# gfacciol/mgm

Measured on AMD Instinct MI355X. Metric: disparity-volumes/sec (W*H*L cost volume -> 8-dir MGM -> WTA+vfit), higher is better.
Workload: dtype f32

## Files before the change

### mgm_amd/csrc/mgm_ctx.hip

```cpp
#include "mgm_host.h"

long long mgm::tune_num(const char *key, long long dflt)
{
#ifdef MGM_HIP_RELEASE
    (void)key;
    return dflt;
#else
    static const std::vector<std::pair<std::string, long long>> table = [] {
        std::vector<std::pair<std::string, long long>> t;
        if (const char *e = getenv("MGM_HIP_TUNE")) {
            std::string s(e);
            size_t i = 0;
            while (i < s.size()) {
                size_t j = s.find(',', i);
                if (j == std::string::npos) j = s.size();
                const std::string item = s.substr(i, j - i);
                const size_t q = item.find('=');
                if (q != std::string::npos && q > 0) t.emplace_back(item.substr(0, q), atoll(item.c_str() + q + 1));
                i = j + 1;
            }
        }
        return t;
    }();
    for (const auto &kv : table)
        if (kv.first == key) return kv.second;
    std::string legacy = "MGM_HIP_";
    for (const char *q = key; *q; q++) legacy += (char)toupper((unsigned char)*q);
    if (const char *e = getenv(legacy.c_str())) return atoll(e);
    return dflt;
#endif
}

const DevSwitches &dev()
{
    static const DevSwitches d = [] {
        auto on = [](const char *n) { return tune_num(n, 1) != 0; };
        return DevSwitches{on("c8"), on("lazy_f32"), on("pad"), (int)tune_num("subv", 1), (int)tune_num("deep", -1),
                           (int)tune_num("wg_per_cu", 0), (int)tune_num("xflags", 0), (int)tune_num("strips", -1), (int)tune_num("xcdq", -1),
                           (int)tune_num("xcdq_k", -1), on("w2"), on("oneb"), 64ll * tune_num("lr_pad", 67)};
    }();
    return d;
}
long long lr_pad_floats() { return dev().lr_pad; }
const WtaSwitches &wta_switches()
{
    static const WtaSwitches w{(int)tune_num("wta_prune_ppw", 2), (int)tune_num("wta_prune_wg", 0), (int)tune_num("wta_wg_per_cu", 0),
                               tune_num("wta_packed", 1) != 0, tune_num("wta_wide4", 1) != 0, tune_num("wta_quad", 1) != 0,
                               (int)tune_num("wta_right_seg", 0)};
    return w;
}

int fail(mgm_ctx *c, int code, const std::string &msg)
{
    if (c) c->err = msg;
    return code;
}
int hipfail(mgm_ctx *c, hipError_t e, const char *what)
{
    (void)hipGetLastError();
    return fail(c, MGM_ERR_HIP, std::string(what) + ": " + hipGetErrorString(e));
}
#define HIPCHK(c, call)                                          \
    do {                                                         \
        hipError_t e__ = (call);                                 \
        if (e__ != hipSuccess) return hipfail((c), e__, #call);  \
    } while (0)

hipError_t dev_malloc(void **p, size_t bytes)
{
    const hipError_t e = hipMalloc(p, bytes);
    if (e != hipSuccess) {
        *p = nullptr;
        (void)hipGetLastError();
    }
    return e;
}

int reserve(mgm_ctx *c, Buf &b, size_t bytes)
{
    if (bytes <= b.cap) return MGM_OK;
    if (b.p) {
        HIPCHK(c, hipStreamSynchronize(c->stream));
        HIPCHK(c, hipFree(b.p));
        b.p = nullptr;
        b.cap = 0;
    }
    hipError_t e = dev_malloc(&b.p, bytes);
    if (e != hipSuccess) {
        return fail(c, MGM_ERR_NOMEM, std::string("hipMalloc(") + std::to_string(bytes) + "): " + hipGetErrorString(e));
    }
    b.cap = bytes;
    return MGM_OK;
}

int ensure_words(mgm_ctx *c)
{
    const void *before = c->words.p;
    if (int r = reserve(c, c->words, sizeof(unsigned) * (size_t)kCtrlWordsTotal)) return r;
    if (c->words.p != before) HIPCHK(c, hipMemsetAsync(c->words.p, 0, c->words.cap, c->stream));
    return MGM_OK;
}
int read_word(mgm_ctx *c, const unsigned *dev, unsigned *out)
{
    HIPCHK(c, hipMemcpyAsync(c->h_words + kHostFlag, dev, sizeof(unsigned), hipMemcpyDeviceToHost, c->stream));
    HIPCHK(c, hipStreamSynchronize(c->stream));
    *out = c->h_words[kHostFlag];
    return MGM_OK;
}

int distance_index(const char *n)
{
    static const char *t[] = {"ad", "sd", "census", "ncc", "btad", "btsd", nullptr};
    int r = 0;
    for (int i = 0; t[i]; i++)
        if (n && !strcmp(n, t[i])) r = i;
    return r;
}
int prefilter_index(const char *n)
{
    static const char *t[] = {"none", "census", "sobelx", "gblur", nullptr};
    int r = 0;
    for (int i = 0; t[i]; i++)
        if (n && !strcmp(n, t[i])) r = i;
    return r;
}
int refinement_index(const char *n)
{
    static const char *t[] = {"none", "vfit", "parabola", "cubic", "parabolaOCV", nullptr};
    int r = 0;
    for (int i = 0; t[i]; i++)
        if (n && !strcmp(n, t[i])) r = i;
    return r;
}

int watch_launch(mgm_ctx *c)
{
    HIPCHK(c, hipMemcpyAsync(c->h_words + kHostWatchdog, ctrl_word(c, kWordWatchdog), sizeof(unsigned), hipMemcpyDeviceToHost, c->stream));
    c->pending_check = true;
    return MGM_OK;
}
int check_watchdog(mgm_ctx *c, bool block)
{
    if (!c->pending_check) return MGM_OK;
    if (block) HIPCHK(c, hipStreamSynchronize(c->stream));
    else if (hipStreamQuery(c->stream) != hipSuccess) return MGM_OK;
    c->pending_check = false;
    if (c->h_words[kHostWatchdog] != 0) {
        c->h_words[kHostWatchdog] = 0;
        if (c->words.p) (void)hipMemsetAsync(ctrl_word(c, kWordWatchdog), 0, sizeof(unsigned), c->stream);
        forget_hand_regions(c);
        return fail(c, MGM_ERR_INTERNAL, "pass kernel watchdog: inter-band hand-off timed out");
    }
    return MGM_OK;
}

bool pipe_uses(const mgm_ctx *c, const void *obj)
{
    if (!c || !obj) return false;
    for (const auto &q : c->pend) {
        for (const mgm_cv *x : q.C) if (x == obj) return true;
        for (const mgm_img *x : q.w8) if (x == obj) return true;
        for (const mgm_img *x : q.out) if (x == obj) return true;
        for (const mgm_img *x : q.outcost) if (x == obj) return true;
    }
    return false;
}

static std::vector<Buf *> workspace_bufs(mgm_ctx *c)
{
    std::vector<Buf *> bufs = {&c->lr, &c->hand.buf, &c->hand2, &c->handm, &c->exact_mins, &c->exact_scratch, &c->census_u, &c->census_v, &c->dbg, &c->stmp, &c->ones8,
                               &c->lr_rel, &c->hand_rel.buf, &c->lmin, &c->wta_stats, &c->wvals, &c->speckle, &c->holes};
    for (int v = 0; v < kMaxBatch; v++) bufs.insert(bufs.end(), {&c->padf[v], &c->pad8[v], &c->wsel[v]});
    return bufs;
}
static void release(Buf &b) { if (b.p) (void)hipFree(b.p), b = Buf{}; }

extern "C" {

const char *mgm_version(void) { return "mgm-hip 0.1 (gfx950)"; }

int mgm_ctx_create(int device, mgm_ctx **out)
{
    if (!out) return MGM_ERR_INVALID;
    *out = nullptr;
    int n = 0;
    if (hipGetDeviceCount(&n) != hipSuccess || n <= 0 || device < 0 || device >= n) return MGM_ERR_HIP;
    if (hipSetDevice(device) != hipSuccess) return MGM_ERR_HIP;
    hipDeviceProp_t prop;
    if (hipGetDeviceProperties(&prop, device) != hipSuccess) return MGM_ERR_HIP;
    if (strncmp(prop.gcnArchName, "gfx950", 6) != 0) return MGM_ERR_HIP;
    mgm_ctx *c = new mgm_ctx();
    c->device = device;
    c->num_cu = prop.multiProcessorCount > 0 ? prop.multiProcessorCount : 256;
    if (hipStreamCreateWithFlags(&c->stream, hipStreamNonBlocking) != hipSuccess) {
        delete c;
        return MGM_ERR_HIP;
    }
    if (hipHostMalloc((void **)&c->h_words, kHostWords * sizeof(unsigned), hipHostMallocDefault) != hipSuccess) {
        (void)hipStreamDestroy(c->stream);
        delete c;
        return MGM_ERR_HIP;
    }
    memset(c->h_words, 0, kHostWords * sizeof(unsigned));
    c->force_build = (int)tune_num("pass_build", 0);
    c->debug_stats = (int)tune_num("debug_stats", 0);
    *out = c;
    return MGM_OK;
}

int mgm_ctx_destroy(mgm_ctx *c)
{
    if (!c) return MGM_OK;
    (void)hipSetDevice(c->device);
    (void)pipe_join(c);
    (void)hipStreamSynchronize(c->stream);
    c->dense_plans.free_all();
    c->rel_plans.free_all();
    for (Buf *b : workspace_bufs(c)) release(*b);
    release(c->words);
    for (auto &t : c->tim) {
        if (t.alias) continue;
        (void)hipEventDestroy(t.a);
        (void)hipEventDestroy(t.b);
    }
    if (c->h_words) (void)hipHostFree(c->h_words);
    (void)hipStreamDestroy(c->stream);
    delete c;
    return MGM_OK;
}

int mgm_ctx_set_pipeline(mgm_ctx *c, int depth)
{
    if (!c) return MGM_ERR_INVALID;
    if (depth < 1 || depth > kMaxBatch) return fail(c, MGM_ERR_INVALID, "mgm_ctx_set_pipeline: depth must be 1..16");
    if (int r = mgm_ctx_synchronize(c)) return r;
    c->pipe_depth = depth;
    return MGM_OK;
}

int mgm_ctx_trim(mgm_ctx *c)
{
    if (int jr = pipe_join(c)) return jr;
    if (!c) return MGM_ERR_INVALID;
    HIPCHK(c, hipSetDevice(c->device));
    if (int r = mgm_ctx_synchronize(c)) return r;
    c->last.clear();
    c->rel_last.clear();
    c->wta_stats_n = 0;
    for (Buf *b : workspace_bufs(c)) release(*b);
    forget_hand_regions(c);
    c->dense_plans.free_all();
    c->rel_plans.free_all();
    return MGM_OK;
}

int mgm_ctx_set_workspace_limit(mgm_ctx *c, unsigned long long bytes)
{
    if (!c) return MGM_ERR_INVALID;
    c->ws_limit = (size_t)bytes;
    return MGM_OK;
}

int mgm_ctx_set_placement_tries(mgm_ctx *c, int tries)
{
    if (!c || tries < 0 || tries > 8) return MGM_ERR_INVALID;
    c->place_tries = tries;
    return MGM_OK;
}

int mgm_ctx_mem_info(mgm_ctx *c, unsigned long long *free_bytes, unsigned long long *total_bytes)
{
    if (!c) return MGM_ERR_INVALID;
    HIPCHK(c, hipSetDevice(c->device));
    size_t f = 0, t = 0;
    HIPCHK(c, hipMemGetInfo(&f, &t));
    if (free_bytes) *free_bytes = f;
    if (total_bytes) *total_bytes = t;
    return MGM_OK;
}

const char *mgm_last_error(const mgm_ctx *c) { return c ? c->err.c_str() : "null context"; }

void *mgm_ctx_stream(mgm_ctx *c) { return c ? (void *)c->stream : nullptr; }

int mgm_ctx_synchronize(mgm_ctx *c)
{
    if (!c) return MGM_ERR_INVALID;
    HIPCHK(c, hipSetDevice(c->device));
    if (int r = pipe_join(c)) return r;
    HIPCHK(c, hipStreamSynchronize(c->stream));
    return check_watchdog(c);
}

int mgm_timing_enable(mgm_ctx *c, int enable)
{
    if (!c) return MGM_ERR_INVALID;
    c->timing = enable != 0;
    return MGM_OK;
}
int mgm_timing_reset(mgm_ctx *c)
{
    if (int jr = pipe_join(c)) return jr;
    if (!c) return MGM_ERR_INVALID;
    (void)hipStreamSynchronize(c->stream);
    for (auto &t : c->tim) {
        if (t.alias) continue;
        (void)hipEventDestroy(t.a);
        (void)hipEventDestroy(t.b);
    }
    c->tim.clear();
    return MGM_OK;
}
int mgm_timing_count(mgm_ctx *c) { return c ? (int)c->tim.size() : 0; }
int mgm_timing_get(mgm_ctx *c, int idx, const char **name, float *ms)
{
    if (!c || idx < 0 || idx >= (int)c->tim.size()) return MGM_ERR_INVALID;
    HIPCHK(c, hipEventSynchronize(c->tim[idx].b));
    float t = 0;
    HIPCHK(c, hipEventElapsedTime(&t, c->tim[idx].a, c->tim[idx].b));
    if (name) *name = c->tim[idx].name;
    if (ms) *ms = t;
    return MGM_OK;
}

int mgm_img_create(mgm_ctx *c, int nx, int ny, int nch, mgm_img **out)
{
    if (!c || !out || nx <= 0 || ny <= 0 || nch <= 0) return fail(c, MGM_ERR_INVALID, "mgm_img_create: bad arguments");
    HIPCHK(c, hipSetDevice(c->device));
    mgm_img *im = new mgm_img{nullptr, nx, ny, nch, c->device};
    hipError_t e = dev_malloc((void **)&im->d, sizeof(float) * (size_t)nx * ny * nch);
    if (e != hipSuccess) {
        delete im;
        return fail(c, MGM_ERR_NOMEM, std::string("mgm_img_create: ") + hipGetErrorString(e));
    }
    *out = im;
    return MGM_OK;
}
int mgm_img_upload(mgm_ctx *c, const float *host, int nx, int ny, int nch, mgm_img **out)
{
    if (!host) return fail(c, MGM_ERR_INVALID, "mgm_img_upload: null host pointer");
    int r = mgm_img_create(c, nx, ny, nch, out);
    if (r) return r;
    hipError_t e = hipMemcpyAsync((*out)->d, host, sizeof(float) * (size_t)nx * ny * nch, hipMemcpyHostToDevice, c->stream);
    if (e == hipSuccess) e = hipStreamSynchronize(c->stream);
    if (e != hipSuccess) {
        r = hipfail(c, e, "mgm_img_upload: copy");
        mgm_img_free(c, *out);
        *out = nullptr;
        return r;
// ... 46 lines not shown
```

### mgm_amd/csrc/mgm_wta.hip

```cpp
#include <algorithm>
#include <cstdlib>

#include "mgm_device.h"
#include "mgm_planner.h"

namespace mgm {

__device__ __forceinline__ void vfit(float v0, float v1, float v2, float &v_min, float &x_min)
{
    if ((v1 > v0) && (v1 > v2)) {
        v_min = v1;
        x_min = 0.0f;
        return;
    }
    float slope = v2 - v1;
    if ((v2 - v1) < (v0 - v1)) slope = v0 - v1;
    x_min = (v0 - v2) / (2.0f * slope);
    v_min = v2 + (x_min - 1.0f) * slope;
}

template <int LPL, int PPW, bool EXACT, int MAXD = kMaxDirs, int SUB = 1>
__global__ void __launch_bounds__(256) k_wta(const WtaParams P)
{
    static_assert(SUB == 1 || EXACT, "several pixels per slab only without padding lanes");
// ... 84 lines not shown
            }
#pragma unroll
            for (int k = 0; k < LPL; k++) {
                const float v = S[k];
                if (o0 + k < Lr_ && (!windowed || (o0 + k >= wl && o0 + k <= wh)) && finite_bits(v) && best > v) {
                    best = v;
                    bi = o0 + k;
                }
            }
#pragma unroll
            for (int d = LANES / 2; d >= 1; d >>= 1) {
                const float ov = __shfl_xor(best, d);
                const int oi = __shfl_xor(bi, d);
                if (ov < best || (ov == best && oi < bi)) {
                    best = ov;
                    bi = oi;
                }
            }
            if (windowed) {
                if (finite_bits(vout)) {
                    if (wl < 0 && wl <= wh && !(best < vout)) {
                        best = vout;
                        bi = wl;
                    }
                    const int hi0 = wl > Lr_ ? wl : Lr_;
                    if (wh >= Lr_ && hi0 <= wh && vout < best) {
                        best = vout;
                        bi = hi0;
                    }
                }
            }
            float outv, outc = best;
            if (bi == 0x7fffffff) outv = __builtin_nanf("");
            else outv = (float)(bi + P.dmin);
            if (P.refine == 1 && !windowed) {
#pragma unroll
                for (int k = 0; k < LPL; k++) sS[wv][m0 + k] = S[k];
                asm volatile("s_waitcnt lgkmcnt(0)" ::: "memory");
                if (bi != 0x7fffffff && bi - 1 >= 0 && bi + 2 <= Lr_ - 1) {
                    const float *sp = sS[wv] + sub * L;
                    const float v0 = sp[bi - 1], v1 = sp[bi], v2 = sp[bi + 1];
                    float vmin, dx;
                    vfit(v0, v1, v2, vmin, dx);
                    outv = (float)(bi + P.dmin) + dx;
                    outc = vmin;
                }
                asm volatile("s_waitcnt lgkmcnt(0)" ::: "memory");
            }
            if (lane % LANES == 0) {
                P.out[pix] = outv;
                P.outcost[pix] = outc;
            }
        }
    }
}

template <int L, int MAXD>
__global__ void __launch_bounds__(256) k_wta_q(const WtaParams P)
{
    static_assert(L == 192 || L == 384, "groups of 768 floats");
    constexpr int NPX = 768 / L;
    constexpr int CPP = L / 4;
    __shared__ float sS[4][768];
    const int wv = threadIdx.x >> 6, lane = threadIdx.x & 63;
    const bool c8 = P.C8 != nullptr;
    const long long ngroup = P.npix / NPX;
    int cpix[3], clab[3];
#pragma unroll
    for (int j = 0; j < 3; j++) {
        const int t = 64 * j + lane;
        cpix[j] = t / CPP;
        clab[j] = (t % CPP) * 4;
    }
    for (long long g = (long long)blockIdx.x * 4 + wv; g < ngroup; g += (long long)gridDim.x * 4) {
        float c[3][4], l[MAXD][3][4];
#pragma unroll
        for (int j = 0; j < 3; j++) {
            if (c8 && P.cbytes == 2) {
                const uint2 w = *reinterpret_cast<const uint2 *>(P.C8 + (g * 768 + 256 * j + 4 * lane) * 2);
                c[j][0] = c16_decode(w.x & 65535u); c[j][1] = c16_decode(w.x >> 16);
                c[j][2] = c16_decode(w.y & 65535u); c[j][3] = c16_decode(w.y >> 16);
            } else if (c8) {
                const unsigned w = *reinterpret_cast<const unsigned *>(P.C8 + g * 768 + 256 * j + 4 * lane);
#pragma unroll
                for (int k = 0; k < 4; k++) c[j][k] = c8_decode((w >> (8 * k)) & 255u);
            } else {
                const float4 q = *reinterpret_cast<const float4 *>(P.C + g * 768 + 256 * j + 4 * lane);
                c[j][0] = q.x; c[j][1] = q.y; c[j][2] = q.z; c[j][3] = q.w;
            }
        }
#pragma unroll
        for (int p = 0; p < MAXD; p++)
            if (p < P.NDIR) {
#pragma unroll
                for (int j = 0; j < 3; j++) {
                    const float4 q = *reinterpret_cast<const float4 *>(P.Lr + (long long)p * P.nvol + g * 768 + 256 * j + 4 * lane);
                    l[p][j][0] = q.x; l[p][j][1] = q.y; l[p][j][2] = q.z; l[p][j][3] = q.w;
                }
            }
        float S[3][4];
        const float f = (float)(P.NDIR - 1);
#pragma unroll
        for (int j = 0; j < 3; j++)
#pragma unroll
            for (int k = 0; k < 4; k++) {
                float a = 0.0f;
#pragma unroll
                for (int p = 0; p < MAXD; p++)
                    if (p < P.NDIR) a = a + l[p][j][k];
                if (P.FIX == 1) a = a - f * c[j][k];
                S[j][k] = a;
            }
        if (P.S) {
#pragma unroll
            for (int j = 0; j < 3; j++) *reinterpret_cast<float4 *>(P.S + g * 768 + 256 * j + 4 * lane) = make_float4(S[j][0], S[j][1], S[j][2], S[j][3]);
        }
        float cb[3];
        int ci[3];
#pragma unroll
        for (int j = 0; j < 3; j++) {
            cb[j] = f_inf();
            ci[j] = 0x7fffffff;
#pragma unroll
            for (int k = 0; k < 4; k++)
                if (finite_bits(S[j][k]) && cb[j] > S[j][k]) {
                    cb[j] = S[j][k];
                    ci[j] = clab[j] + k;
                }
        }
        if (P.refine == 1) {
#pragma unroll
            for (int j = 0; j < 3; j++) *reinterpret_cast<float4 *>(&sS[wv][256 * j + 4 * lane]) = make_float4(S[j][0], S[j][1], S[j][2], S[j][3]);
        }
#pragma unroll
        for (int q = 0; q < NPX; q++) {
            float best = f_inf();
            int bi = 0x7fffffff;
#pragma unroll
            for (int j = 0; j < 3; j++)
                if (cpix[j] == q && (cb[j] < best)) {
                    best = cb[j];
                    bi = ci[j];
                }
#pragma unroll
            for (int d = 32; d >= 1; d >>= 1) {
                const float ov = __shfl_xor(best, d);
                const int oi = __shfl_xor(bi, d);
                if (ov < best || (ov == best && oi < bi)) {
                    best = ov;
                    bi = oi;
                }
            }
            float outv, outc = best;
            if (bi == 0x7fffffff) outv = __builtin_nanf("");
            else outv = (float)(bi + P.dmin);
            if (P.refine == 1) {
                asm volatile("s_waitcnt lgkmcnt(0)" ::: "memory");
                if (bi != 0x7fffffff && bi - 1 >= 0 && bi + 2 <= L - 1) {
                    const float *sp = sS[wv] + q * L;
                    float vmin, dx;
                    vfit(sp[bi - 1], sp[bi], sp[bi + 1], vmin, dx);
                    outv = (float)(bi + P.dmin) + dx;
                    outc = vmin;
                }
            }
            if (lane == 0) {
                P.out[g * NPX + q] = outv;
                P.outcost[g * NPX + q] = outc;
            }
        }
        if (P.refine == 1) asm volatile("s_waitcnt lgkmcnt(0)" ::: "memory");
    }
}

__global__ void __launch_bounds__(256) k_wta_any(const WtaParams P)
{
    const int wv = threadIdx.x >> 6, lane = threadIdx.x & 63;
    const int L = P.L, Lr_ = P.Lreal;
    const float f = (float)(P.NDIR - 1);
    float vout = 0.0f;
    if (P.FIX == 1) vout = vout - f * f_inf();
    for (long long pix = (long long)blockIdx.x * 4 + wv; pix < P.npix; pix += (long long)gridDim.x * 4) {
        int cl = 0, ch = Lr_ - 1;
        if (P.clo) {
            cl = (int)P.clo[pix] - P.dmin;
            ch = (int)P.chi[pix] - P.dmin;
        }
        const bool windowed = P.wlo != nullptr;
        int wl = 0, wh = 0;
        if (windowed) {
            wl = (int)P.wlo[pix] - P.dmin;
            wh = (int)P.whi[pix] - P.dmin;
        }
        auto S_at = [&](int o) {
            float a = 0.0f;
            for (int p = 0; p < P.NDIR; p++) a = a + P.Lr[(long long)p * P.nvol + pix * L + o];
            if (P.FIX == 1)
                a = a - f * (!P.C8 ? P.C[pix * L + o]
                                   : (P.cbytes == 2 ? c16_decode(reinterpret_cast<const unsigned short *>(P.C8)[pix * L + o]) : c8_decode(P.C8[pix * L + o])));
            if (o < cl || o > ch) a = vout;
            return a;
        };
        float best = f_inf();
        int bi = 0x7fffffff;
        for (int o = lane; o < Lr_; o += 64) {
            const float v = S_at(o);
            if (P.S) P.S[pix * Lr_ + o] = v;
            if ((!windowed || (o >= wl && o <= wh)) && finite_bits(v) && best > v) {
                best = v;
                bi = o;
            }
        }
#pragma unroll
        for (int d = 32; d >= 1; d >>= 1) {
            const float ov = __shfl_xor(best, d);
            const int oi = __shfl_xor(bi, d);
            if (ov < best || (ov == best && oi < bi)) {
                best = ov;
                bi = oi;
            }
        }
        if (windowed && finite_bits(vout)) {
            if (wl < 0 && wl <= wh && !(best < vout)) {
                best = vout;
                bi = wl;
            }
            const int hi0 = wl > Lr_ ? wl : Lr_;
            if (wh >= Lr_ && hi0 <= wh && vout < best) {
                best = vout;
                bi = hi0;
            }
        }
        float outv, outc = best;
        if (bi == 0x7fffffff) outv = __builtin_nanf("");
        else outv = (float)(bi + P.dmin);
        if (P.refine == 1 && !windowed && bi != 0x7fffffff && bi - 1 >= 0 && bi + 2 <= Lr_ - 1) {
            float vmin, dx;
            vfit(S_at(bi - 1), S_at(bi), S_at(bi + 1), vmin, dx);
            outv = (float)(bi + P.dmin) + dx;
            outc = vmin;
        }
        if (lane == 0) {
            P.out[pix] = outv;
            P.outcost[pix] = outc;
        }
    }
}

template <int MAXD, int K>
__device__ __forceinline__ void sum_fix(const float (&l)[MAXD][K], const float (&c)[K], int ndir, int fix, float (&S)[K])
{
#pragma unroll
    for (int k = 0; k < K; k++) S[k] = 0.0f;
#pragma unroll
    for (int p = 0; p < MAXD; p++)
        if (p < ndir) {
#pragma unroll
            for (int k = 0; k < K; k++) S[k] = S[k] + l[p][k];
        }
    if (fix == 1) {
        const float f = (float)(ndir - 1);
#pragma unroll
        for (int k = 0; k < K; k++) S[k] = S[k] - f * c[k];
    }
}
template <int CTRL>
__device__ __forceinline__ float dpp_f(float v)
{
    return __builtin_bit_cast(float, __builtin_amdgcn_update_dpp(0, __builtin_bit_cast(int, v), CTRL, 0xf, 0xf, false));
}
template <int CTRL>
__device__ __forceinline__ float dpp_fmin(float v)
{
    return __builtin_fminf(v, dpp_f<CTRL>(v));
}
__device__ __forceinline__ float group_fmin(float v)
{
    v = dpp_fmin<0xB1>(v);
    v = dpp_fmin<0x4E>(v);
    return dpp_fmin<0x141>(v);
}
template <int CTRL>
__device__ __forceinline__ void dpp_take(float &best, int &bi)
{
    const float ov = dpp_f<CTRL>(best);
    const int oi = __builtin_amdgcn_update_dpp(0, bi, CTRL, 0xf, 0xf, false);
    if (ov < best || (ov == best && oi < bi)) {
        best = ov;
        bi = oi;
    }
}
template <int PPW, int ND>
__device__ __forceinline__ void wta_pruned(const WtaParams &P)
{
    constexpr int MAXD = ND;
    constexpr int L = 256;
    constexpr int NONE = 0x7fffffff;
    const int wv = threadIdx.x >> 6, lane = threadIdx.x & 63;
    const int j = lane & 7;
    const int gsh = lane & ~7;
    const int ndir = ND, fix = P.FIX;
    const long long mstride = P.nvol / 32;
    unsigned nloaded = 0, npx = 0;
    for (long long g0 = ((long long)blockIdx.x * 4 + wv) * (8 * PPW); g0 < P.npix; g0 += (long long)gridDim.x * 4 * 8 * PPW) {
        long long pix[PPW];
        bool own[PPW];
        uint4 cq[PPW][2];
        float mn[PPW][MAXD];
#pragma unroll
        for (int u = 0; u < PPW; u++) {
            const long long q = g0 + 8 * u + (lane >> 3);
            own[u] = q < P.npix;
            pix[u] = own[u] ? q : P.npix - 1;
            const uint4 *cp = reinterpret_cast<const uint4 *>(P.C8 + pix[u] * L + j * 32);
            cq[u][0] = cp[0], cq[u][1] = cp[1];
#pragma unroll
            for (int p = 0; p < MAXD; p++)
                if (p < ndir) mn[u][p] = P.Lmin[(long long)p * mstride + pix[u] * (L / 32) + j];
        }
        float clb[PPW];
        int seed[PPW];
#pragma unroll
        for (int u = 0; u < PPW; u++) {
            const unsigned w[8] = {cq[u][0].x, cq[u][0].y, cq[u][0].z, cq[u][0].w, cq[u][1].x, cq[u][1].y, cq[u][1].z, cq[u][1].w};
            unsigned m = 0;
#pragma unroll
            for (int i = 0; i < 8; i++)
#pragma unroll
                for (int k = 0; k < 4; k++) m = max(m, (((w[i] >> (8 * k)) & 255u) + 1u) & 255u);
            float lm[MAXD][1], LB[1];
            const float cm[1] = {(float)((int)m - 1)};
#pragma unroll
            for (int p = 0; p < MAXD; p++) lm[p][0] = p < ndir ? mn[u][p] : 0.0f;
            sum_fix<MAXD>(lm, cm, ndir, fix, LB);
            const float lb = (m != 0u && LB[0] == LB[0]) ? LB[0] : f_inf();
            clb[u] = lb;
            const float gmin = group_fmin(lb);
            const unsigned at = (unsigned)(__builtin_amdgcn_ballot_w64(lb == gmin) >> gsh) & 255u;
            seed[u] = gmin < f_inf() ? __builtin_ctz(at | 256u) : -1;
        }
        auto chunk_S = [&](const int (&ck)[PPW], float (&S)[PPW][4]) {
            float l[PPW][MAXD][4];
            unsigned cw[PPW];
#pragma unroll
            for (int u = 0; u < PPW; u++) {
                const long long at = pix[u] * L + ck[u] * 32 + j * 4;
                cw[u] = *reinterpret_cast<const unsigned *>(P.C8 + at);
#pragma unroll
                for (int p = 0; p < MAXD; p++)
                    if (p < ndir) {
                        const float4 q = *reinterpret_cast<const float4 *>(P.Lr + (long long)p * P.nvol + at);
                        l[u][p][0] = q.x, l[u][p][1] = q.y, l[u][p][2] = q.z, l[u][p][3] = q.w;
                    }
            }
#pragma unroll
            for (int u = 0; u < PPW; u++) {
                float c[4];
#pragma unroll
                for (int k = 0; k < 4; k++) c[k] = c8_decode((cw[u] >> (8 * k)) & 255u);
                sum_fix<MAXD>(l[u], c, ndir, fix, S[u]);
            }
        };
        float best[PPW];
        int bi[PPW], sck[PPW];
        unsigned cand[PPW];
        {
            float S[PPW][4];
#pragma unroll
            for (int u = 0; u < PPW; u++) sck[u] = seed[u] > 0 ? seed[u] : 0;
            chunk_S(sck, S);
#pragma unroll
            for (int u = 0; u < PPW; u++) {
                best[u] = f_inf();
                bi[u] = NONE;
                if (seed[u] >= 0) {
#pragma unroll
                    for (int k = 0; k < 4; k++)
                        if (finite_bits(S[u][k]) && best[u] > S[u][k]) {
                            best[u] = S[u][k];
                            bi[u] = seed[u] * 32 + j * 4 + k;
                        }
                }
                const float best0 = group_fmin(best[u]);
                const bool cd = seed[u] >= 0 && j != seed[u] && clb[u] <= best0;
                const unsigned long long cdm = __builtin_amdgcn_ballot_w64(cd);
                cand[u] = (unsigned)(cdm >> gsh) & 255u;
                const unsigned long long ownm = __builtin_amdgcn_ballot_w64(own[u]);
                nloaded += (unsigned)__builtin_popcountll(cdm & ownm) + (unsigned)__builtin_popcountll(__builtin_amdgcn_ballot_w64(own[u] && j == seed[u]));
                npx += (unsigned)__builtin_popcountll(ownm) >> 3;
            }
        }
        for (;;) {
            bool more = false;
#pragma unroll
            for (int u = 0; u < PPW; u++) more = more || cand[u] != 0u;
            if (!__builtin_amdgcn_ballot_w64(more)) break;
            if (more) {
                int ck[PPW];
                float S[PPW][4];
#pragma unroll
                for (int u = 0; u < PPW; u++) ck[u] = cand[u] != 0u ? __builtin_ctz(cand[u]) : sck[u];
                chunk_S(ck, S);
#pragma unroll
                for (int u = 0; u < PPW; u++)
                    if (cand[u] != 0u) {
#pragma unroll
                        for (int k = 0; k < 4; k++) {
                            const int o = ck[u] * 32 + j * 4 + k;
                            if (finite_bits(S[u][k]) && (S[u][k] < best[u] || (S[u][k] == best[u] && o < bi[u]))) {
                                best[u] = S[u][k];
                                bi[u] = o;
                            }
                        }
                        cand[u] &= cand[u] - 1u;
                    }
            }
        }
#pragma unroll
        for (int u = 0; u < PPW; u++) {
            dpp_take<0xB1>(best[u], bi[u]);
            dpp_take<0x4E>(best[u], bi[u]);
            dpp_take<0x141>(best[u], bi[u]);
            const int b = bi[u];
            float outv, outc = best[u];
            if (b == NONE) outv = __builtin_nanf("");
            else outv = (float)(b + P.dmin);
            if (P.refine == 1) {
                const bool gate = b != NONE && b - 1 >= 0 && b + 2 <= L - 1;
                float a = 0.0f;
                if (gate && j < 3) {
                    const long long at = pix[u] * L + (b - 1 + j);
#pragma unroll
                    for (int p = 0; p < MAXD; p++)
                        if (p < ndir) a = a + P.Lr[(long long)p * P.nvol + at];
                    if (fix == 1) a = a - (float)(ndir - 1) * c8_decode(P.C8[at]);
                }
                const float v1 = dpp_f<0xB1>(a), v2 = dpp_f<0x4E>(a);
                if (gate) {
                    float vmin, dx;
                    vfit(a, v1, v2, vmin, dx);
                    outv = (float)(b + P.dmin) + dx;
                    outc = vmin;
                }
            }
            if (j == 0 && own[u]) {
                P.out[pix[u]] = outv;
                P.outcost[pix[u]] = outc;
            }
        }
    }
    if (P.stats && lane == 0) atomicAdd(P.stats + (blockIdx.x & 63) * 16, ((unsigned long long)npx << 32) | nloaded);
}
template <int PPW, int MAXD, bool ALLD>
__global__ void __launch_bounds__(256) k_wta_pruned(const WtaParams P)
{
    if constexpr (ALLD) {
        wta_pruned<PPW, MAXD>(P);
    } else {
#define ND_CASE(N_)                                         \
    case N_:                                                \
        if constexpr (N_ < MAXD) wta_pruned<PPW, N_>(P);    \
        break;
        switch (P.NDIR) {
            ND_CASE(1) ND_CASE(2) ND_CASE(3) ND_CASE(4) ND_CASE(5) ND_CASE(6) ND_CASE(7)
            default: break;
        }
#undef ND_CASE
    }
}

static_assert(kWtaWidestLabels == kMaxLPL * 64, "plan_wta sends wider volumes to k_wta_any");
hipError_t launch_wta(const WtaParams &p, const WtaChoice &c, hipStream_t s)
{
    const dim3 grid((unsigned)c.grid), block(256);
#define WTA(LPL_, PPW_, EXACT_, MAXD_, SUB_)                                                                     \
    if (c.LPL == LPL_ && c.PPW == PPW_ && c.EXACT == EXACT_ && c.MAXD == MAXD_ && c.SUB == SUB_) {               \
        hipLaunchKernelGGL((k_wta<LPL_, PPW_, EXACT_ != 0, MAXD_, SUB_>), grid, block, 0, s, p);                 \
        return hipGetLastError();                                                                                \
    }
#define WTA_Q(LPL_, MAXD_)                                                                                       \
    if (c.LPL == LPL_ && c.MAXD == MAXD_) {                                                                      \
        hipLaunchKernelGGL((k_wta_q<64 * LPL_, MAXD_>), grid, block, 0, s, p);                                   \
        return hipGetLastError();                                                                                \
    }
#define WTA_PRUNED(PPW_, MAXD_, ALLD_)                                                                           \
    if (c.PPW == PPW_ && c.MAXD == MAXD_ && c.ALLD == ALLD_ && p.NDIR >= 1 && (ALLD_ ? p.NDIR == MAXD_ : p.NDIR < MAXD_)) { \
        hipLaunchKernelGGL((k_wta_pruned<PPW_, MAXD_, ALLD_ != 0>), grid, block, 0, s, p);                       \
        return hipGetLastError();                                                                                \
    }
    switch (c.family) {
        case kWtaPruned:
            if (!p.Lmin) break;
            WTA_PRUNED(2, 8, 1) WTA_PRUNED(1, 8, 1) WTA_PRUNED(2, 4, 1) WTA_PRUNED(1, 4, 1) WTA_PRUNED(1, 4, 0) WTA_PRUNED(1, 8, 0)
            break;
        case kWtaAny:
            hipLaunchKernelGGL(k_wta_any, grid, block, 0, s, p);
            return hipGetLastError();
        case kWtaQuad:
            WTA_Q(3, 4) WTA_Q(3, 8) WTA_Q(6, 4) WTA_Q(6, 8)
            break;
        case kWtaPacked:
            WTA(4, 4, 1, 4, 2) WTA(4, 2, 1, 8, 2) WTA(4, 4, 1, 4, 4) WTA(4, 2, 1, 8, 4)
            break;
        case kWtaPlain:
            WTA(1, 8, 1, 4, 1) WTA(1, 4, 1, 8, 1) WTA(1, 1, 0, 8, 1)
            WTA(2, 8, 1, 4, 1) WTA(2, 4, 1, 8, 1) WTA(2, 1, 0, 8, 1)
            WTA(3, 4, 1, 4, 1) WTA(3, 2, 1, 8, 1) WTA(3, 1, 0, 8, 1)
            WTA(4, 6, 1, 4, 1) WTA(4, 3, 1, 8, 1) WTA(4, 1, 0, 8, 1)
            WTA(6, 2, 1, 4, 1) WTA(6, 1, 1, 8, 1) WTA(6, 1, 0, 8, 1)
            WTA(8, 2, 1, 4, 1) WTA(8, 1, 1, 8, 1) WTA(8, 1, 0, 8, 1)
            WTA(12, 1, 1, 8, 1) WTA(12, 1, 0, 8, 1)
            WTA(16, 1, 1, 8, 1) WTA(16, 1, 0, 8, 1)
            WTA(24, 1, 0, 8, 1)
            WTA(32, 1, 0, 8, 1)
            break;
        default: break;
    }
#undef WTA
#undef WTA_Q
#undef WTA_PRUNED
    return hipErrorInvalidValue;
}

__device__ __forceinline__ void parabolafit(const float (&v)[4], float &v_min, float &x_min)
{
    if (v[1] > v[0] && v[1] > v[2]) {
        x_min = 0;
        v_min = v[1];
        return;
    }
    const float c = v[1];
    const float b = (v[2] - v[0]) / 2;
    const float a = (v[2] - 2 * v[1] + v[0]) / 2;
    float x = -b / (2 * a);
    if (x > 1) x = 1;
    if (x < -1) x = -1;
    v_min = (a * x + b) * x + c;
    x_min = x;
}

__device__ __forceinline__ void parabolafit_ocv(const float (&v)[4], float &v_min, float &x_min)
{
    if (v[1] > v[0] && v[1] > v[2]) {
        x_min = 0;
        v_min = v[1];
        return;
    }
    const float c = v[1];
    float b = (v[2] - v[0]) / 2;
    float a = (v[2] - 2 * v[1] + v[0]) / 2;
    a *= 2;
    b *= 2;
    a = a > 1.0 ? a : 1.0;
    float x = (-b + a) / (2 * a);
    if (x > 1) x = 1;
    if (x < -1) x = -1;
    v_min = (a * x + b) * x + c;
    x_min = x;
}

__device__ __forceinline__ float cubic_interp(const float (&p)[4], const float x)
{
    return p[1] + 0.5 * x *
                      (p[2] - p[0] + x * (2.0 * p[0] - 5.0 * p[1] + 4.0 * p[2] - p[3] + x * (3.0 * (p[1] - p[2]) + p[3] - p[0])));
}

__device__ __forceinline__ void cubicfit(const float (&p)[4], float &out_pmin, float &out_xmin)
{
    float pmin, xmin;
    if (p[1] < p[2]) {
        pmin = p[1];
        xmin = 0.0;
    } else {
        pmin = p[2];
        xmin = 1.0;
    }
    const double a = 0.5 * 3.0 * (3.0 * (p[1] - p[2]) + p[3] - p[0]);
    const double b = 2.0 * p[0] - 5.0 * p[1] + 4.0 * p[2] - p[3];
    const double c = 0.5 * (p[2] - p[0]);
    const double discr = b * b - 4.0 * a * c;
    if (discr >= 0) {
        const double z1 = (-b + __builtin_sqrt(discr)) / (2.0 * a);
        const double z2 = (-b - __builtin_sqrt(discr)) / (2.0 * a);
        if (z1 > 0.0 && z1 < 1.0) {
            const float tmp = cubic_interp(p, z1);
            if (tmp < pmin) {
                pmin = tmp;
                xmin = z1;
            }
        }
        if (z2 > 0.0 && z2 < 1.0) {
            const float tmp = cubic_interp(p, z2);
            if (tmp < pmin) {
                pmin = tmp;
                xmin = z2;
            }
        }
    }
    out_pmin = pmin;
    out_xmin = xmin;
}

template <int SPL, int CB>
__global__ void __launch_bounds__(256) k_wta_rel(const WtaRelParams P)
{
    constexpr int SLOTS = 16 * SPL;
    const int wv = threadIdx.x >> 6, lane = threadIdx.x & 63, li = lane & 15, grp = lane >> 4;
    const float f = (float)(P.NDIR - 1);
    float vout = 0.0f;
    if (P.FIX == 1) vout = vout - f * f_inf();
    const bool vfin = finite_bits(vout);
    const long long nquads = (P.npix + 3) / 4;
    for (long long q4 = (long long)blockIdx.x * 4 + wv; q4 < nquads; q4 += (long long)gridDim.x * 4) {
        const long long pix0 = q4 * 4 + grp;
        const bool live = pix0 < P.npix;
        const long long pix = live ? pix0 : P.npix - 1;
        const int4 rec = reinterpret_cast<const int4 *>(P.base)[pix];
        const int b = rec.x, lo = rec.y, hi = rec.z;
        const bool windowed = P.wlo != nullptr;
        const int wl = windowed ? (int)P.wlo[pix] : lo, wh = windowed ? (int)P.whi[pix] : hi;
        typedef float f4 __attribute__((ext_vector_type(4)));
        float a[SPL];
#pragma unroll
        for (int q = 0; q < SPL; q++) a[q] = 0.0f;
        for (int p = 0; p < P.NDIR; p++) {
#pragma unroll
            for (int h = 0; h < SPL / 4; h++) {
                const f4 t = reinterpret_cast<const f4 *>(P.Lr + (long long)p * P.nvol + pix * SLOTS + SPL * li)[h];
#pragma unroll
                for (int q = 0; q < 4; q++) a[4 * h + q] = a[4 * h + q] + t[q];
            }
        }
        if (P.FIX == 1) {
            constexpr int NWORD = SPL * CB / 4;
            unsigned cw[NWORD];
#pragma unroll
            for (int w = 0; w < NWORD; w++) cw[w] = reinterpret_cast<const unsigned *>(P.c8 + (pix * SLOTS + SPL * li) * CB)[w];
#pragma unroll
            for (int q = 0; q < SPL; q++)
                a[q] = a[q] - f * (CB == 1 ? c8_decode((cw[q / 4] >> (8 * (q % 4))) & 255u)
                                           : (CB == 2 ? c16_decode((cw[q / 2] >> (16 * (q % 2))) & 65535u) : __builtin_bit_cast(float, cw[q * CB / 4])));
        }
        float val[SPL];
        float cb = f_inf();
        int ci = 0x7fffffff;
#pragma unroll
        for (int q = 0; q < SPL; q++) {
            const int d = b + SPL * li + q;
            const bool own = d >= lo && d <= hi;
            val[q] = own ? a[q] : vout;
            if (own && d >= wl && d <= wh && finite_bits(val[q]) && val[q] < cb) {
                cb = val[q];
                ci = d;
            }
        }
        dpp_take<0xB1>(cb, ci);
        dpp_take<0x4E>(cb, ci);
        dpp_take<0x141>(cb, ci);
        dpp_take<0x140>(cb, ci);
        float best = f_inf();
        int bi = 0x7fffffff;
        if (wl < lo && wl <= wh && vfin) {
            best = vout;
            bi = wl;
        }
        if (ci != 0x7fffffff && best > cb) {
            best = cb;
            bi = ci;
        }
        const int hi0 = wl > hi + 1 ? wl : hi + 1;
        if (wh > hi && hi0 <= wh && vfin && vout < best) {
            best = vout;
            bi = hi0;
        }
        float outv, outc = best;
        if (bi == 0x7fffffff) outv = __builtin_nanf("");
        else outv = (float)bi;
        float v[4];
#pragma unroll
        for (int k = 0; k < 4; k++) {
            const int sl = (bi == 0x7fffffff ? b : bi) - 1 + k - b;
            const int e = sl & (SPL - 1);
            float mine = val[0];
#pragma unroll
            for (int q = 1; q < SPL; q++) mine = e == q ? val[q] : mine;
            const float x = __shfl(mine, (lane & 48) | ((sl / SPL) & 15));
            v[k] = (sl >= 0 && sl < SLOTS) ? x : vout;
        }
        if (P.refine >= 1 && bi != 0x7fffffff && bi - 1 >= wl && bi + 2 <= wh) {
            float vmin = outc, dx = 0;
            if (P.refine == 1) vfit(v[0], v[1], v[2], vmin, dx);
            else if (P.refine == 2) parabolafit(v, vmin, dx);
            else if (P.refine == 3) cubicfit(v, vmin, dx);
            else parabolafit_ocv(v, vmin, dx);
            outv = (float)bi + dx;
            outc = vmin;
        }
        if (li == 0 && live) {
            P.out[pix] = outv;
            P.outcost[pix] = outc;
        }
    }
}
__global__ void __launch_bounds__(256) k_rel_S(const WtaRelParams P, long long n, int L, int dmin, float *__restrict__ S)
{
    const long long t = (long long)blockIdx.x * blockDim.x + threadIdx.x;
    if (t >= n) return;
    const long long pix = t / L;
    const int d = dmin + (int)(t - pix * L);
    const int4 rec = reinterpret_cast<const int4 *>(P.base)[pix];
    const float f = (float)(P.NDIR - 1);
    float s = f_inf();
    if (d >= rec.y && d <= rec.z) {
        const long long k = pix * P.slots + (d - rec.x);
        s = 0.0f;
        for (int p = 0; p < P.NDIR; p++) s = s + P.Lr[(long long)p * P.nvol + k];
        if (P.FIX == 1)
            s = s - f * (P.cb == 1 ? c8_decode((unsigned)P.c8[k])
                                   : (P.cb == 2 ? c16_decode((unsigned)reinterpret_cast<const uint16_t *>(P.c8)[k]) : reinterpret_cast<const float *>(P.c8)[k]));
    } else if (P.FIX == 1)
        s = s - f * f_inf();
    S[t] = s;
}
hipError_t launch_rel_S(const WtaRelParams &p, int L, int dmin, float *S, hipStream_t s)
{
    const long long n = p.npix * L;
    hipLaunchKernelGGL(k_rel_S, dim3((unsigned)((n + 255) / 256)), dim3(256), 0, s, p, n, L, dmin, S);
    return hipGetLastError();
}
hipError_t launch_wta_rel(const WtaRelParams &p, hipStream_t s)
{
    const WtaRelChoice c = plan_wta_rel(WtaRelRequest{p.npix, p.num_cu, p.slots, p.cb});
    const dim3 grid((unsigned)c.grid);
#define WTA_REL(SPL_, CB_)                                                                \
    if (c.SPL == SPL_ && c.CB == CB_) {                                                   \
        hipLaunchKernelGGL((k_wta_rel<SPL_, CB_>), grid, dim3(256), 0, s, p);             \
        return hipGetLastError();                                                         \
    }
    WTA_REL(8, 4) WTA_REL(8, 2) WTA_REL(8, 1) WTA_REL(4, 4) WTA_REL(4, 2) WTA_REL(4, 1)
#undef WTA_REL
    return hipErrorInvalidValue;
}

__global__ void __launch_bounds__(256) k_refine(const float *__restrict__ S, long long npix, int L, int dmin, int method,
                                                const float *__restrict__ wlo, const float *__restrict__ whi, float vout,
                                                float *__restrict__ out, float *__restrict__ outcost)
{
    const long long i = (long long)blockIdx.x * blockDim.x + threadIdx.x;
// ... 389 lines not shown
```

Before: 177.6.

## Prefetch next pixel group and double-buffer candidate chunk loads in pruned WTA

The pruned WTA kernel now loads the next pixel group's packed costs and per-chunk minima before processing the current group. For one pixel per slab, candidate chunk loads are double-buffered so the next chunk's aggregated costs load while the current one is summed. Subpixel refinement reuses neighbour sums captured during the argmin and only refetches across chunk boundaries, with the winning lane writing the output. The default pixels-per-slab drops from 2 to 1 to use the pipelined path. The cost is more register pressure from two buffers and a prefetch slot, which may lower occupancy.

```diff
diff --git a/mgm_amd/csrc/mgm_ctx.hip b/mgm_amd/csrc/mgm_ctx.hip
--- a/mgm_amd/csrc/mgm_ctx.hip
+++ b/mgm_amd/csrc/mgm_ctx.hip
@@ -44,7 +44,7 @@
 long long lr_pad_floats() { return dev().lr_pad; }
 const WtaSwitches &wta_switches()
 {
-    static const WtaSwitches w{(int)tune_num("wta_prune_ppw", 2), (int)tune_num("wta_prune_wg", 0), (int)tune_num("wta_wg_per_cu", 0),
+    static const WtaSwitches w{(int)tune_num("wta_prune_ppw", 1),(int)tune_num("wta_prune_wg", 0), (int)tune_num("wta_wg_per_cu", 0),
                                tune_num("wta_packed", 1) != 0, tune_num("wta_wide4", 1) != 0, tune_num("wta_quad", 1) != 0,
                                (int)tune_num("wta_right_seg", 0)};
     return w;
diff --git a/mgm_amd/csrc/mgm_wta.hip b/mgm_amd/csrc/mgm_wta.hip
--- a/mgm_amd/csrc/mgm_wta.hip
+++ b/mgm_amd/csrc/mgm_wta.hip
@@ -410,21 +410,30 @@
     const int ndir = ND, fix = P.FIX;
     const long long mstride = P.nvol / 32;
     unsigned nloaded = 0, npx = 0;
-    for (long long g0 = ((long long)blockIdx.x * 4 + wv) * (8 * PPW); g0 < P.npix; g0 += (long long)gridDim.x * 4 * 8 * PPW) {
+    const long long turn = (long long)gridDim.x * 4 * 8 * PPW;
+    long long g0 = ((long long)blockIdx.x * 4 + wv) * (8 * PPW);
+    uint4 cq[PPW][2];
+    float mn[PPW][MAXD];
+    auto load_a = [&](const long long g) {
+#pragma unroll
+        for (int u = 0; u < PPW; u++) {
+            const long long q = g + 8 * u + (lane >> 3), px = q < P.npix ? q : P.npix - 1;
+            const uint4 *cp = reinterpret_cast<const uint4 *>(P.C8 + px * L + j * 32);
+            cq[u][0] = cp[0], cq[u][1] = cp[1];
+#pragma unroll
+            for (int p = 0; p < MAXD; p++)
+                if (p < ndir) mn[u][p] = P.Lmin[(long long)p * mstride + px * (L / 32) + j];
+        }
+    };
+    if (g0 < P.npix) load_a(g0);
+    for (; g0 < P.npix; g0 += turn) {
         long long pix[PPW];
         bool own[PPW];
-        uint4 cq[PPW][2];
-        float mn[PPW][MAXD];
 #pragma unroll
         for (int u = 0; u < PPW; u++) {
             const long long q = g0 + 8 * u + (lane >> 3);
             own[u] = q < P.npix;
             pix[u] = own[u] ? q : P.npix - 1;
-            const uint4 *cp = reinterpret_cast<const uint4 *>(P.C8 + pix[u] * L + j * 32);
-            cq[u][0] = cp[0], cq[u][1] = cp[1];
-#pragma unroll
-            for (int p = 0; p < MAXD; p++)
-                if (p < ndir) mn[u][p] = P.Lmin[(long long)p * mstride + pix[u] * (L / 32) + j];
         }
         float clb[PPW];
         int seed[PPW];
@@ -447,9 +456,8 @@
             const unsigned at = (unsigned)(__builtin_amdgcn_ballot_w64(lb == gmin) >> gsh) & 255u;
             seed[u] = gmin < f_inf() ? __builtin_ctz(at | 256u) : -1;
         }
-        auto chunk_S = [&](const int (&ck)[PPW], float (&S)[PPW][4]) {
-            float l[PPW][MAXD][4];
-            unsigned cw[PPW];
+        if (g0 + turn < P.npix) load_a(g0 + turn);
+        auto chunk_load =[&](const int (&ck)[PPW], float (&l)[PPW][MAXD][4], unsigned (&cw)[PPW]) {
 #pragma unroll
             for (int u = 0; u < PPW; u++) {
                 const long long at = pix[u] * L + ck[u] * 32 + j * 4;
@@ -461,6 +469,8 @@
                         l[u][p][0] = q.x, l[u][p][1] = q.y, l[u][p][2] = q.z, l[u][p][3] = q.w;
                     }
             }
+        };
+        auto chunk_sum = [&](const float (&l)[PPW][MAXD][4], const unsigned (&cw)[PPW], float (&S)[PPW][4]) {
 #pragma unroll
             for (int u = 0; u < PPW; u++) {
                 float c[4];
@@ -468,10 +478,30 @@
                 for (int k = 0; k < 4; k++) c[k] = c8_decode((cw[u] >> (8 * k)) & 255u);
                 sum_fix<MAXD>(l[u], c, ndir, fix, S[u]);
             }
+        };
+        auto chunk_S = [&](const int (&ck)[PPW], float (&S)[PPW][4]) {
+            float l[PPW][MAXD][4];
+            unsigned cw[PPW];
+            chunk_load(ck, l, cw);
+            chunk_sum(l, cw, S);
         };
         float best[PPW];
         int bi[PPW], sck[PPW];
         unsigned cand[PPW];
+        float nlo[PPW], nhi[PPW];
+        auto take = [&](const int u, const float (&S)[4], const int ck, const bool ties) {
+            const float lo = dpp_f<0x111>(S[3]), hi = dpp_f<0x101>(S[0]);
+#pragma unroll
+            for (int k = 0; k < 4; k++) {
+                const int o = ck * 32 + j * 4 + k;
+                if (finite_bits(S[k]) && (S[k] < best[u] || (ties && S[k] == best[u] && o < bi[u]))) {
+                    best[u] = S[k];
+                    bi[u] = o;
+                    nlo[u] = k > 0 ? S[k > 0 ? k - 1 : 0] : lo;
+                    nhi[u] = k < 3 ? S[k < 3 ? k + 1 : 3] : hi;
+                }
+            }
+        };
         {
             float S[PPW][4];
 #pragma unroll
@@ -481,14 +511,8 @@
             for (int u = 0; u < PPW; u++) {
                 best[u] = f_inf();
                 bi[u] = NONE;
-                if (seed[u] >= 0) {
-#pragma unroll
-                    for (int k = 0; k < 4; k++)
-                        if (finite_bits(S[u][k]) && best[u] > S[u][k]) {
-                            best[u] = S[u][k];
-                            bi[u] = seed[u] * 32 + j * 4 + k;
-                        }
-                }
+                nlo[u] = nhi[u] = 0.0f;
+                if (seed[u] >= 0) take(u, S[u], seed[u], false);
                 const float best0 = group_fmin(best[u]);
                 const bool cd = seed[u] >= 0 && j != seed[u] && clb[u] <= best0;
                 const unsigned long long cdm = __builtin_amdgcn_ballot_w64(cd);
@@ -498,60 +522,95 @@
                 npx += (unsigned)__builtin_popcountll(ownm) >> 3;
             }
         }
-        for (;;) {
-            bool more = false;
-#pragma unroll
-            for (int u = 0; u < PPW; u++) more = more || cand[u] != 0u;
-            if (!__builtin_amdgcn_ballot_w64(more)) break;
-            if (more) {
-                int ck[PPW];
+        if constexpr (PPW == 1) {
+            float lA[PPW][MAXD][4], lB[PPW][MAXD][4];
+            unsigned cwA[PPW], cwB[PPW];
+            int ckA[PPW], ckB[PPW];
+            bool actA[PPW], actB[PPW];
+            auto issue = [&](int (&ck)[PPW], bool (&act)[PPW], float (&l)[PPW][MAXD][4], unsigned (&cw)[PPW]) {
+                bool more = false;
+#pragma unroll
+                for (int u = 0; u < PPW; u++) {
+                    act[u] = cand[u] != 0u;
+                    ck[u] = act[u] ? __builtin_ctz(cand[u]) : sck[u];
+                    cand[u] &= cand[u] - 1u;
+                    more = more || act[u];
+                }
+                if (!__builtin_amdgcn_ballot_w64(more)) return false;
+                if (more) chunk_load(ck, l, cw);
+                return true;
+            };
+            auto consume = [&](const int (&ck)[PPW], const bool (&act)[PPW], const float (&l)[PPW][MAXD][4], const unsigned (&cw)[PPW]) {
                 float S[PPW][4];
-#pragma unroll
-                for (int u = 0; u < PPW; u++) ck[u] = cand[u] != 0u ? __builtin_ctz(cand[u]) : sck[u];
-                chunk_S(ck, S);
+                chunk_sum(l, cw, S);
 #pragma unroll
                 for (int u = 0; u < PPW; u++)
-                    if (cand[u] != 0u) {
-#pragma unroll
-                        for (int k = 0; k < 4; k++) {
-                            const int o = ck[u] * 32 + j * 4 + k;
-                            if (finite_bits(S[u][k]) && (S[u][k] < best[u] || (S[u][k] == best[u] && o < bi[u]))) {
-                                best[u] = S[u][k];
-                                bi[u] = o;
-                            }
+                    if (act[u]) take(u, S[u], ck[u], true);
+            };
+            if (issue(ckA, actA, lA, cwA))
+                for (;;) {
+                    const bool nb = issue(ckB, actB, lB, cwB);
+                    consume(ckA, actA, lA, cwA);
+                    if (!nb) break;
+                    const bool na = issue(ckA, actA, lA, cwA);
+                    consume(ckB, actB, lB, cwB);
+                    if (!na) break;
+                }
+        } else {
+            for (;;) {
+                bool more = false;
+#pragma unroll
+                for (int u = 0; u < PPW; u++) more = more || cand[u] != 0u;
+                if (!__builtin_amdgcn_ballot_w64(more)) break;
+                if (more) {
+                    int ck[PPW];
+                    float S[PPW][4];
+#pragma unroll
+                    for (int u = 0; u < PPW; u++) ck[u] = cand[u] != 0u ? __builtin_ctz(cand[u]) : sck[u];
+                    chunk_S(ck, S);
+#pragma unroll
+                    for (int u = 0; u < PPW; u++)
+                        if (cand[u] != 0u) {
+                            take(u, S[u], ck[u], true);
+                            cand[u] &= cand[u] - 1u;
                         }
-                        cand[u] &= cand[u] - 1u;
-                    }
+                }
             }
         }
 #pragma unroll
         for (int u = 0; u < PPW; u++) {
+            const int mine = bi[u];
             dpp_take<0xB1>(best[u], bi[u]);
             dpp_take<0x4E>(best[u], bi[u]);
             dpp_take<0x141>(best[u], bi[u]);
             const int b = bi[u];
+            const bool writer = b == NONE ? j == 0 : mine == b;
             float outv, outc = best[u];
             if (b == NONE) outv = __builtin_nanf("");
             else outv = (float)(b + P.dmin);
             if (P.refine == 1) {
                 const bool gate = b != NONE && b - 1 >= 0 && b + 2 <= L - 1;
-                float a = 0.0f;
-                if (gate && j < 3) {
-                    const long long at = pix[u] * L + (b - 1 + j);
-#pragma unroll
-                    for (int p = 0; p < MAXD; p++)
-                        if (p < ndir) a = a + P.Lr[(long long)p * P.nvol + at];
-                    if (fix == 1) a = a - (float)(ndir - 1) * c8_decode(P.C8[at]);
-                }
-                const float v1 = dpp_f<0xB1>(a), v2 = dpp_f<0x4E>(a);
+                const bool below = (b & 31) == 0, fetch = writer && gate && (below || (b & 31) == 31);
+                if (__builtin_amdgcn_ballot_w64(fetch)) {
+                    if (fetch) {
+                        const long long at = pix[u] * L + (below ? b - 1 : b + 1);
+                        float a = 0.0f;
+#pragma unroll
+                        for (int p = 0; p < MAXD; p++)
+                            if (p < ndir) a = a + P.Lr[(long long)p * P.nvol + at];
+                        if (fix == 1) a = a - (float)(ndir - 1) * c8_decode(P.C8[at]);
+                        if (below) nlo[u] = a;
+                        else nhi[u] = a;
+                    }
+                }
                 if (gate) {
                     float vmin, dx;
-                    vfit(a, v1, v2, vmin, dx);
+                    vfit(nlo[u], best[u], nhi[u], vmin, dx);
                     outv = (float)(b + P.dmin) + dx;
                     outc = vmin;
                 }
             }
-            if (j == 0 && own[u]) {
+            if (writer && own[u]) {
                 P.out[pix[u]] = outv;
                 P.outcost[pix[u]] = outc;
             }
```

Result: faster. 189.3 (median of 6 runs) (+6.6%).
